# JamesKane/DecodingUsTools

Measured on AMD Instinct MI355X. Metric: reference bases classified/sec (whole node) + BED bit-exact vs CPU ref, higher is better.
Workload: dtype u8 (quality bytes thresholded to pass bits on the host, counted bit-sliced on the device); 1 GPU; coverage -L chr21 synthetic 30x 150bp paired, device-resident, one contig per GPU; contig_len=46709983, reads_per_contig=9076994, aligned_bases_per_contig=1361549100, parallelism=contig-per-gpu x1, options=cli defaults (4,500,10,20,10,1,0.1)

## Files before the change

### decodingustools_amd/csrc/pileup_rows.hip.h

```cpp
#pragma once
#include "kernels.hip.h"

namespace clk {

template <bool HEAD4> struct HeadOf { typedef uint2 type; };
template <> struct HeadOf<true> { typedef uint32_t type; };
template <bool HEAD4> __device__ __forceinline__ typename HeadOf<HEAD4>::type head_at(const void *heads, uint32_t r)
{
    return reinterpret_cast<const typename HeadOf<HEAD4>::type *>(heads)[r];
}
struct HeadCand { uint32_t cb, ce, low; bool hit; };
template <int T> __device__ __forceinline__ HeadCand head_cand(const uint2 h, uint32_t W)
{
    const uint32_t x = h.x, span = h.y & kHeadSpanMax, e = x + span;
    return HeadCand{x > W ? x - W : 0u, e - W, h.y >> 31, span && e > W && x < W + (uint32_t)T};
}
template <int T> __device__ __forceinline__ HeadCand head_cand(const uint32_t h, uint32_t W)
{
    const int32_t span = (int32_t)((h >> 16) & 0x7FFFu), dx = (int32_t)(int16_t)(uint16_t)(h - W), e = dx + span;
    return HeadCand{(uint32_t)(dx > 0 ? dx : 0), (uint32_t)e, h >> 31, span && e > 0 && dx < T};
}

typedef unsigned int RowWords __attribute__((ext_vector_type(4)));
constexpr uint32_t kRowNoUnit = 0x80000000u;
struct RowLane { __amdgpu_buffer_rsrc_t rs; uint32_t off; int32_t n; };
__device__ __forceinline__ RowLane row_lane(const uint4 *rows, const WinMeta &wm, uint32_t lane, uint32_t g0)
{
    const uint32_t s = lane >> 3;
    uint32_t n = wm.rn, first = s * wm.rn, units = 8u * wm.rn;
    if (wm.q0) {
        n = (uint32_t)(wm.q0 >> (8u * s)) & 0xFFu;
        const unsigned long long below = wm.q0 & ((1ull << (8u * s)) - 1ull);
        first = __builtin_amdgcn_sad_u8((uint32_t)below, 0u, __builtin_amdgcn_sad_u8((uint32_t)(below >> 32), 0u, 0u));
        const uint32_t lo = (uint32_t)wm.q0, hi = (uint32_t)(wm.q0 >> 32);
        const uint32_t f = (lo & 0x00FF00FFu) + ((lo >> 8) & 0x00FF00FFu) + (hi & 0x00FF00FFu) + ((hi >> 8) & 0x00FF00FFu);
        units = (f + (f >> 16)) & 0xFFFFu;
    }
    return RowLane{__builtin_amdgcn_make_buffer_rsrc(const_cast<uint4 *>(rows + (size_t)wm.rlo * 8u), 0, (int)(units * 128u), 0x00020000),
                   (first + g0) * 128u + (lane & 7u) * 16u, (int32_t)(n - g0)};
}
__device__ __forceinline__ uint4 row_unit(const RowLane &rl, int k)
{
    const RowWords v = __builtin_amdgcn_raw_buffer_load_b128(rl.rs, (k < rl.n ? rl.off : kRowNoUnit) + (uint32_t)k * 128u, 0, 0);
    return make_uint4(v.x, v.y, v.z, v.w);
}
__device__ __forceinline__ void row_advance(RowLane &rl, int by) { rl.off += (uint32_t)by * 128u; rl.n -= by; }
typedef unsigned int HeadWords __attribute__((ext_vector_type(2)));
template <bool HEAD4> __device__ __forceinline__ typename HeadOf<HEAD4>::type head_fetch(__amdgpu_buffer_rsrc_t rs, uint32_t off);
template <> __device__ __forceinline__ uint32_t head_fetch<true>(__amdgpu_buffer_rsrc_t rs, uint32_t off)
{
    return __builtin_amdgcn_raw_buffer_load_b32(rs, off, 0, 0);
}
template <> __device__ __forceinline__ uint2 head_fetch<false>(__amdgpu_buffer_rsrc_t rs, uint32_t off)
{
    const HeadWords v = __builtin_amdgcn_raw_buffer_load_b64(rs, off, 0, 0);
    return make_uint2(v.x, v.y);
}

__device__ __forceinline__ uint32_t bs_maj(uint32_t a, uint32_t b, uint32_t c) { return (a & b) | (c & (a | b)); }

template <int NP>
__device__ __forceinline__ void bs_add4(uint32_t (&c)[NP], const uint4 x)
{
    const uint32_t t0 = c[0] ^ x.x ^ x.y, k0 = bs_maj(c[0], x.x, x.y);
    c[0] = t0 ^ x.z ^ x.w;
    const uint32_t k1 = bs_maj(t0, x.z, x.w);
    uint32_t k = bs_maj(c[1], k0, k1);
    c[1] = c[1] ^ k0 ^ k1;
#pragma unroll
    for (int p = 2; p < NP; ++p) { const uint32_t t = c[p] & k; c[p] ^= k; k = t; }
}

template <int NP>
__device__ __forceinline__ uint32_t bs_less_than(const uint32_t (&c)[NP], unsigned long long K)
{
    if (NP < 64 && (K >> NP) != 0ull) return 0xFFFFFFFFu;
    uint32_t lt = 0u, eq = 0xFFFFFFFFu;
#pragma unroll
    for (int p = NP - 1; p >= 0; --p) {
        if ((K >> p) & 1ull) { lt |= eq & ~c[p]; eq &= c[p]; }
        else eq &= ~c[p];
    }
    return lt;
}

struct RowsArgs {
    const uint4    *rows;
    const void     *heads;
    const uint32_t *wide_idx;
    const WinMeta  *win;
    const uint32_t *refn;
    const uint32_t *lut8;
    uint16_t       *runs;
    uint8_t        *first_state, *last_state;
    WinPartial     *winpart;
    uint32_t        extent, n_win, n_win8;
    uint32_t        min_depth, max_depth;
    uint32_t        min_depth_for_low_mapq;
    const uint32_t *lut;
    double          max_low_mapq_fraction;
    uint8_t        *state;
    uint32_t       *dbg_raw, *dbg_qc, *dbg_low;
};

constexpr int kRowsBlock = 64;
constexpr int rows_min_waves(bool DEBUG, bool DEEP, int NP)
{
    return ((DEEP || NP > 16) ? 3 : (NP > 8 ? 4 : 5)) - (DEBUG ? 1 : 0);
}
template <int T, bool DEBUG, bool DEEP, int NP, bool HEAD4>
__global__ __launch_bounds__(kRowsBlock, rows_min_waves(DEBUG, DEEP, NP)) void k_pileup_rows(RowsArgs a)
{
    constexpr int kBlock = kRowsBlock;
    constexpr int PER = T / kBlock;
    static_assert(PER == 32 && T == 2048 && kBlock == 64, "a lane owns a block of 32 positions: T = 64 x 32, one wave");
    constexpr int kDiffWords = DEEP ? T : T / 2;
    constexpr int G = 12;
    __shared__ __attribute__((aligned(16))) uint32_t s_raw[kDiffWords];
    __shared__ __attribute__((aligned(16))) uint32_t s_low[kDiffWords];
#ifdef CL_ROWS_LDS_PAD
    __shared__ uint32_t s_pad[CL_ROWS_LDS_PAD / 4];
    s_pad[threadIdx.x] = threadIdx.x;
#endif

    const uint32_t w = (blockIdx.x & 7u) * a.n_win8 + (blockIdx.x >> 3);
    if (w >= a.n_win) return;
    const uint32_t lane = threadIdx.x;
    const uint32_t W = w * (uint32_t)T;
    const uint32_t p0 = W + lane * PER;

    const WinMeta wm = a.win[w];
    const uint32_t lo = wm.lo, hi = wm.hi, wlo = wm.wlo, wn = wm.wn;
    const uint32_t n_cand = wn + (hi - lo);
    const uint32_t ng = wm.rn;
    RowLane rl = row_lane(a.rows, wm, lane, 0u);

    uint4 rv[G];
#pragma unroll
    for (int j = 0; j < G; ++j) rv[j] = row_unit(rl, j);
    constexpr int U = 8;
    typedef typename HeadOf<HEAD4>::type Head;
    const __amdgpu_buffer_rsrc_t hrs = __builtin_amdgcn_make_buffer_rsrc(
        const_cast<char *>(static_cast<const char *>(a.heads) + (size_t)lo * sizeof(Head)), 0, (int)((hi - lo) * (uint32_t)sizeof(Head)), 0x00020000);
    auto load_heads = [&](uint32_t base, Head (&hh)[U]) {
#pragma unroll
        for (int u = 0; u < U; ++u) {
            const uint32_t o = base + (uint32_t)u * kBlock + lane - wn;
            hh[u] = head_fetch<HEAD4>(hrs, o < hi - lo ? o * (uint32_t)sizeof(Head) : 0xFFFFFFF0u);
        }
        if (wn > base) {
#pragma unroll
            for (int u = 0; u < U; ++u) {
                const uint32_t v = base + (uint32_t)u * kBlock + lane;
                if (v < wn) {
                    const uint32_t r = a.wide_idx[wlo + v];
                    __builtin_assume(r < (1u << 29));
                    hh[u] = head_at<HEAD4>(a.heads, r);
                }
            }
        }
    };
    Head hh[U];
    load_heads(0u, hh);
    const uint32_t wlut = a.lut8[lane];
    const uint32_t refn = a.refn[(size_t)w * (T / 32) + lane];

    {
        const uint4 z = make_uint4(0, 0, 0, 0);
        uint4 *r4 = reinterpret_cast<uint4 *>(s_raw), *l4 = reinterpret_cast<uint4 *>(s_low);
        const uint4 zb = DEEP ? z : make_uint4(0x8000u, 0x8000u, 0x8000u, 0x8000u);
#pragma unroll
        for (int i = 0; i < kDiffWords / 4 / kBlock; ++i) { r4[i * kBlock + lane] = zb; l4[i * kBlock + lane] = zb; }
    }
    __syncthreads();

    uint32_t c[NP];
#pragma unroll
    for (int p = 0; p < NP; ++p) c[p] = 0u;
    if (ng) {
        for (uint32_t g0 = 0; g0 < ng; g0 += (uint32_t)G) {
#pragma unroll
            for (int j = 0; j < G; ++j) {
                if (g0 + (uint32_t)j < ng) bs_add4<NP>(c, rv[j]);
            }
            if (g0 + (uint32_t)G < ng) {
                row_advance(rl, G);
#pragma unroll
                for (int j = 0; j < G; ++j) rv[j] = row_unit(rl, j);
            }
        }
    }
    for (uint32_t base = 0;;) {
#pragma unroll
        for (int u = 0; u < U; ++u) {
            const HeadCand hc = head_cand<T>(hh[u], W);
            if (hc.hit) {
                const uint32_t cb = hc.cb, ce = hc.ce;
                uint32_t ib, vb, ie, ve2;
                if (DEEP) { ib = cb; vb = 1u; ie = ce; ve2 = 0xFFFFFFFFu; }
                else {
                    ib = cb >> 1; vb = (cb & 1u) ? 0x10000u : 1u;
                    ie = ce >> 1; ve2 = (ce & 1u) ? 0xFFFF0000u : 0xFFFFFFFFu;
                }
                atomicAdd(&s_raw[ib], vb);
                if (ce < (uint32_t)T) atomicAdd(&s_raw[ie], ve2);
                if (hc.low) {
                    atomicAdd(&s_low[ib], vb);
                    if (ce < (uint32_t)T) atomicAdd(&s_low[ie], ve2);
                }
            }
        }
        base += (uint32_t)U * kBlock;
        if (base >= n_cand) break;
        load_heads(base, hh);
    }
    __syncthreads();

    const uint32_t ltb = bs_less_than<NP>(c, (unsigned long long)a.min_depth);
    const uint32_t gtb = a.max_depth > 0u ? ~bs_less_than<NP>(c, (unsigned long long)a.max_depth + 1ull) : 0u;
    unsigned long long nbits = 0;
#pragma unroll
    for (int p = 0; p < NP; ++p) nbits += (unsigned long long)__popc(c[p]) << p;

    constexpr int NH = DEEP ? 1 : PER / 2;
    uint32_t xr[NH], xl[NH];
    uint32_t tr = 0, tl = 0;
    if constexpr (DEEP) {
        xr[0] = xl[0] = 0u;
#pragma unroll
        for (int q = 0; q < PER / 4; ++q) {
            const uint4 x = reinterpret_cast<const uint4 *>(s_raw)[lane * (PER / 4) + q];
            const uint4 y = reinterpret_cast<const uint4 *>(s_low)[lane * (PER / 4) + q];
            tr += x.x + x.y + x.z + x.w; tl += y.x + y.y + y.z + y.w;
        }
    } else {
#pragma unroll
        for (int q = 0; q < NH / 4; ++q) {
            const uint4 x = reinterpret_cast<const uint4 *>(s_raw)[lane * (NH / 4) + q];
            const uint4 y = reinterpret_cast<const uint4 *>(s_low)[lane * (NH / 4) + q];
            xr[4 * q] = x.x; xr[4 * q + 1] = x.y; xr[4 * q + 2] = x.z; xr[4 * q + 3] = x.w;
            xl[4 * q] = y.x; xl[4 * q + 1] = y.y; xl[4 * q + 2] = y.z; xl[4 * q + 3] = y.w;
        }
#pragma unroll
        for (int h = 0; h < NH; ++h) {
            tr = __builtin_amdgcn_sad_u16(xr[h], 0u, tr);
            tl = __builtin_amdgcn_sad_u16(xl[h], 0u, tl);
        }
        tr = (uint32_t)(int32_t)(int16_t)(uint16_t)tr; tl = (uint32_t)(int32_t)(int16_t)(uint16_t)tl;
    }
    const uint32_t offr = dpp_incl_scan_u32(tr) - tr, offl = dpp_incl_scan_u32(tl) - tl;

    uint32_t covb = 0, lowb = 0, mx = 0;
    if constexpr (!DEEP) {
        uint32_t sr = offr, sl = offl, ncov = 0, nlow = 0;
        constexpr int B = 8;
#pragma unroll
        for (int g = 0; g < PER; g += B) {
            uint32_t r8[B], l8[B], t8[B];
#pragma unroll
            for (int k = 0; k < B; ++k) {
                const int i = g + k;
                sr += (i & 1) ? (uint32_t)((int32_t)xr[i / 2] >> 16) : (xr[i / 2] & 0xFFFFu) - 0x8000u;
                sl += (i & 1) ? (uint32_t)((int32_t)xl[i / 2] >> 16) : (xl[i / 2] & 0xFFFFu) - 0x8000u;
                r8[k] = sr; l8[k] = sl;
                t8[k] = (uint32_t)__builtin_amdgcn_ds_bpermute((int)(sr & ~3u), (int)wlut);
            }
#pragma unroll
            for (int k = 0; k < B; ++k) {
                mx = r8[k] > mx ? r8[k] : mx;
                const uint32_t thr = __builtin_amdgcn_ubfe(t8[k], r8[k] << 3, 8u);
                ncov = __builtin_amdgcn_alignbit(ncov, r8[k] - 1u, 31);
                nlow = __builtin_amdgcn_alignbit(nlow, l8[k] - thr, 31);
                if (DEBUG) {
                    if (a.dbg_raw) a.dbg_raw[p0 + g + k] = r8[k];
                    if (a.dbg_low) a.dbg_low[p0 + g + k] = l8[k];
                }
            }
        }
        covb = ~__builtin_bitreverse32(ncov); lowb = ~__builtin_bitreverse32(nlow);
    }
    if (DEEP || mx >= 255u) {
        const uint32_t mdl = a.min_depth_for_low_mapq < 0x7FFFFFFFu ? a.min_depth_for_low_mapq : 0x7FFFFFFFu;
        uint32_t sr = offr, sl = offl, ncov = 0, nlow = 0;
        mx = 0;
#pragma unroll 1
        for (int h = 0; h < PER / 2; ++h) {
            uint32_t dr[2], dl[2];
            if (DEEP) {
                dr[0] = s_raw[lane * PER + 2 * h]; dr[1] = s_raw[lane * PER + 2 * h + 1];
                dl[0] = s_low[lane * PER + 2 * h]; dl[1] = s_low[lane * PER + 2 * h + 1];
            } else {
                const uint32_t xr = s_raw[lane * (PER / 2) + h], xl = s_low[lane * (PER / 2) + h];
                dr[0] = (xr & 0xFFFFu) - 0x8000u; dr[1] = (uint32_t)((int32_t)xr >> 16);
                dl[0] = (xl & 0xFFFFu) - 0x8000u; dl[1] = (uint32_t)((int32_t)xl >> 16);
            }
#pragma unroll
            for (int k = 0; k < 2; ++k) {
                sr += dr[k]; sl += dl[k];
                const uint32_t raw = sr, low = sl;
                mx = raw > mx ? raw : mx;
                uint32_t thr = a.lut[raw < kLutSize ? raw : kLutSize - 1u];
                thr = thr < 0x7FFFFFFFu ? thr : 0x7FFFFFFFu;
                thr |= (uint32_t)((int32_t)(raw - mdl) >> 31) >> 1;
                uint32_t d = low - thr;
                if (raw >= kLutSize) {
                    const bool is_low = raw >= a.min_depth_for_low_mapq && ((double)low / (double)raw) > a.max_low_mapq_fraction;
                    d = is_low ? 0u : 0x80000000u;
                }
                ncov = __builtin_amdgcn_alignbit(ncov, raw - 1u, 31);
                nlow = __builtin_amdgcn_alignbit(nlow, d, 31);
                if (DEBUG) {
                    if (a.dbg_raw) a.dbg_raw[p0 + 2 * h + k] = raw;
                    if (a.dbg_low) a.dbg_low[p0 + 2 * h + k] = low;
                }
            }
        }
        covb = ~__builtin_bitreverse32(ncov); lowb = ~__builtin_bitreverse32(nlow);
    }
    const uint32_t n_ok = p0 >= a.extent ? 0u : (a.extent - p0 < (uint32_t)PER ? a.extent - p0 : (uint32_t)PER);
    const uint32_t okb = n_ok >= (uint32_t)PER ? 0xFFFFFFFFu : ((1u << n_ok) - 1u);
    const uint32_t Nk = refn & okb, notN = ~refn & okb, covk = covb & okb;
    const uint32_t t0 = notN & covk;
    const uint32_t rLow = t0 & lowb, t1 = t0 & ~lowb;
    const uint32_t rLT = t1 & ltb, t2 = t1 & ~ltb;
    const uint32_t rGT = t2 & gtb, rC = t2 & ~gtb;
    const uint32_t rNC = notN & ~covk;
    const uint32_t s0 = rC | rLT | rLow, s1 = rNC | rLT, s2 = rGT | rLow;
    auto state_at = [&](uint32_t j) -> uint32_t { return ((s0 >> j) & 1u) | (((s1 >> j) & 1u) << 1) | (((s2 >> j) & 1u) << 2); };
    if (DEBUG) {
#pragma unroll 1
        for (uint32_t i = 0; i < (uint32_t)PER; ++i) {
            uint32_t qc = 0;
#pragma unroll
            for (int p = 0; p < NP; ++p) qc |= ((c[p] >> i) & 1u) << p;
            if (a.dbg_qc) a.dbg_qc[p0 + i] = qc;
            a.state[p0 + i] = (uint8_t)(((okb >> i) & 1u) ? state_at(i) : 0xFFu);
        }
    }
    const uint32_t last_st = state_at((uint32_t)PER - 1u);
    const uint32_t below = (uint32_t)__shfl_up((int)last_st, 1);
    const uint32_t pv = lane > 0 ? below : state_at(0u);
    const uint32_t bnd = ((s0 ^ ((s0 << 1) | (pv & 1u))) | (s1 ^ ((s1 << 1) | ((pv >> 1) & 1u))) | (s2 ^ ((s2 << 1) | (pv >> 2)))) & okb;
    const uint32_t nb = __popc(bnd);
    {
        const uint32_t inc = dpp_incl_scan_u32(nb);
        if (nb) {
            uint16_t *dst = a.runs + (size_t)w * T + (inc - nb);
            for (uint32_t m = bnd; m; m &= m - 1u) {
                const uint32_t j = (uint32_t)__ffs((int)m) - 1u;
                *dst++ = (uint16_t)((lane * PER + j) | (state_at(j) << 12));
            }
        }
        if (lane == 0) a.first_state[w] = (uint8_t)state_at(0u);
        if (lane == kBlock - 1) a.last_state[w] = (uint8_t)last_st;
    }
    static_assert(sizeof(WinPartial) == 96 && offsetof(WinPartial, sum_reflen) == 72 && offsetof(WinPartial, n_inner) == 88 &&
                  offsetof(WinPartial, max_raw) == 92, "WinPartial as twelve 8-byte words");
    {
        const uint32_t pk0 = dpp_wave_sum_u32(__popc(Nk) | (__popc(rC) << 16));
        const uint32_t pk1 = dpp_wave_sum_u32(__popc(rNC) | (__popc(rLT) << 16));
        const uint32_t pk2 = dpp_wave_sum_u32(__popc(rGT) | (__popc(rLow) << 16));
        const uint32_t pk3 = dpp_wave_sum_u32(__popc(covk) | (nb << 16));
        const unsigned long long qc = NP <= 16 ? (unsigned long long)dpp_wave_sum_u32((uint32_t)nbits) : wave_sum_u64(nbits);
        mx = dpp_wave_max_u32(mx);
        const uint32_t f[12] = {pk0 & 0xFFFFu, pk0 >> 16, pk1 & 0xFFFFu, pk1 >> 16, pk2 & 0xFFFFu, pk2 >> 16,
                                pk3 & 0xFFFFu, (uint32_t)qc, 0u, 0u, 0u, pk3 >> 16};
        if (lane < 12u) {
            uint32_t vlo = 0u;
#pragma unroll
            for (uint32_t k = 0; k < 12u; ++k) vlo = lane == k ? f[k] : vlo;
            const uint32_t vhi = lane == 7u ? (uint32_t)(qc >> 32) : (lane == 11u ? mx : 0u);
            reinterpret_cast<unsigned long long *>(a.winpart + w)[lane] = (unsigned long long)vlo | ((unsigned long long)vhi << 32);
        }
    }
}

}
```

Before: 758.8 billion bases/s.

## Pack raw and low-MAPQ diffs into one word and use CSA tree counters

```diff
diff --git a/decodingustools_amd/csrc/pileup_rows.hip.h b/decodingustools_amd/csrc/pileup_rows.hip.h
--- a/decodingustools_amd/csrc/pileup_rows.hip.h
+++ b/decodingustools_amd/csrc/pileup_rows.hip.h
@@ -69,6 +69,37 @@
     c[1] = c[1] ^ k0 ^ k1;
 #pragma unroll
     for (int p = 2; p < NP; ++p) { const uint32_t t = c[p] & k; c[p] ^= k; k = t; }
+}
+
+__device__ __forceinline__ uint32_t bs_csa(uint32_t &s, uint32_t a, uint32_t b)
+{
+    const uint32_t k = bs_maj(s, a, b);
+    s ^= a ^ b;
+    return k;
+}
+template <int NP>
+__device__ __forceinline__ void bs_ripple(uint32_t (&c)[NP], int from, uint32_t k)
+{
+#pragma unroll
+    for (int p = from; p < NP; ++p) { const uint32_t t = c[p] & k; c[p] ^= k; k = t; }
+}
+template <int NP>
+__device__ __forceinline__ void bs_add8(uint32_t (&c)[NP], const uint4 x, const uint4 y)
+{
+    static_assert(NP >= 4, "the tree of 8 rows ends in plane 2");
+    const uint32_t a0 = bs_csa(c[0], x.x, x.y), a1 = bs_csa(c[0], x.z, x.w), a2 = bs_csa(c[0], y.x, y.y), a3 = bs_csa(c[0], y.z, y.w);
+    const uint32_t b0 = bs_csa(c[1], a0, a1), b1 = bs_csa(c[1], a2, a3);
+    bs_ripple<NP>(c, 3, bs_csa(c[2], b0, b1));
+}
+template <int NP>
+__device__ __forceinline__ void bs_add16(uint32_t (&c)[NP], const uint4 x, const uint4 y, const uint4 z, const uint4 v)
+{
+    static_assert(NP >= 5, "the tree of 16 rows ends in plane 3");
+    const uint32_t a0 = bs_csa(c[0], x.x, x.y), a1 = bs_csa(c[0], x.z, x.w), a2 = bs_csa(c[0], y.x, y.y), a3 = bs_csa(c[0], y.z, y.w);
+    const uint32_t a4 = bs_csa(c[0], z.x, z.y), a5 = bs_csa(c[0], z.z, z.w), a6 = bs_csa(c[0], v.x, v.y), a7 = bs_csa(c[0], v.z, v.w);
+    const uint32_t b0 = bs_csa(c[1], a0, a1), b1 = bs_csa(c[1], a2, a3), b2 = bs_csa(c[1], a4, a5), b3 = bs_csa(c[1], a6, a7);
+    const uint32_t d0 = bs_csa(c[2], b0, b1), d1 = bs_csa(c[2], b2, b3);
+    bs_ripple<NP>(c, 4, bs_csa(c[3], d0, d1));
 }
 
 template <int NP>
@@ -106,7 +137,7 @@
 constexpr int kRowsBlock = 64;
 constexpr int rows_min_waves(bool DEBUG, bool DEEP, int NP)
 {
-    return ((DEEP || NP > 16) ? 3 : (NP > 8 ? 4 : 5)) - (DEBUG ? 1 : 0);
+    return ((DEEP || NP > 16) ? 3 : (NP > 8 ? 4 : 5)) - (DEBUG ? (!DEEP && NP <= 8 ? 2 : 1) : 0);
 }
 template <int T, bool DEBUG, bool DEEP, int NP, bool HEAD4>
 __global__ __launch_bounds__(kRowsBlock, rows_min_waves(DEBUG, DEEP, NP)) void k_pileup_rows(RowsArgs a)
@@ -114,10 +145,9 @@
     constexpr int kBlock = kRowsBlock;
     constexpr int PER = T / kBlock;
     static_assert(PER == 32 && T == 2048 && kBlock == 64, "a lane owns a block of 32 positions: T = 64 x 32, one wave");
-    constexpr int kDiffWords = DEEP ? T : T / 2;
     constexpr int G = 12;
-    __shared__ __attribute__((aligned(16))) uint32_t s_raw[kDiffWords];
-    __shared__ __attribute__((aligned(16))) uint32_t s_low[kDiffWords];
+    __shared__ __attribute__((aligned(16))) uint32_t s_diff[DEEP ? 2 * T : T];
+    uint32_t *const s_raw = s_diff, *const s_low = s_diff + T;
 #ifdef CL_ROWS_LDS_PAD
     __shared__ uint32_t s_pad[CL_ROWS_LDS_PAD / 4];
     s_pad[threadIdx.x] = threadIdx.x;
@@ -166,11 +196,9 @@
     const uint32_t refn = a.refn[(size_t)w * (T / 32) + lane];
 
     {
-        const uint4 z = make_uint4(0, 0, 0, 0);
-        uint4 *r4 = reinterpret_cast<uint4 *>(s_raw), *l4 = reinterpret_cast<uint4 *>(s_low);
-        const uint4 zb = DEEP ? z : make_uint4(0x8000u, 0x8000u, 0x8000u, 0x8000u);
-#pragma unroll
-        for (int i = 0; i < kDiffWords / 4 / kBlock; ++i) { r4[i * kBlock + lane] = zb; l4[i * kBlock + lane] = zb; }
+        uint4 *d4 = reinterpret_cast<uint4 *>(s_diff);
+#pragma unroll
+        for (int i = 0; i < (DEEP ? 2 * T : T) / 4 / kBlock; ++i) d4[i * kBlock + lane] = make_uint4(0, 0, 0, 0);
     }
     __syncthreads();
 
@@ -180,8 +208,9 @@
     if (ng) {
         for (uint32_t g0 = 0; g0 < ng; g0 += (uint32_t)G) {
 #pragma unroll
-            for (int j = 0; j < G; ++j) {
-                if (g0 + (uint32_t)j < ng) bs_add4<NP>(c, rv[j]);
+            for (int j = 0; j < G; j += 4) {
+                if (g0 + (uint32_t)j + 2u < ng) bs_add16<NP>(c, rv[j], rv[j + 1], rv[j + 2], rv[j + 3]);
+                else if (g0 + (uint32_t)j < ng) bs_add8<NP>(c, rv[j], rv[j + 1]);
             }
             if (g0 + (uint32_t)G < ng) {
                 row_advance(rl, G);
@@ -196,17 +225,17 @@
             const HeadCand hc = head_cand<T>(hh[u], W);
             if (hc.hit) {
                 const uint32_t cb = hc.cb, ce = hc.ce;
-                uint32_t ib, vb, ie, ve2;
-                if (DEEP) { ib = cb; vb = 1u; ie = ce; ve2 = 0xFFFFFFFFu; }
-                else {
-                    ib = cb >> 1; vb = (cb & 1u) ? 0x10000u : 1u;
-                    ie = ce >> 1; ve2 = (ce & 1u) ? 0xFFFF0000u : 0xFFFFFFFFu;
-                }
-                atomicAdd(&s_raw[ib], vb);
-                if (ce < (uint32_t)T) atomicAdd(&s_raw[ie], ve2);
-                if (hc.low) {
-                    atomicAdd(&s_low[ib], vb);
-                    if (ce < (uint32_t)T) atomicAdd(&s_low[ie], ve2);
+                if (DEEP) {
+                    atomicAdd(&s_raw[cb], 1u);
+                    if (ce < (uint32_t)T) atomicAdd(&s_raw[ce], 0xFFFFFFFFu);
+                    if (hc.low) {
+                        atomicAdd(&s_low[cb], 1u);
+                        if (ce < (uint32_t)T) atomicAdd(&s_low[ce], 0xFFFFFFFFu);
+                    }
+                } else {
+                    const uint32_t v = 1u + (hc.low << 16);
+                    atomicAdd(&s_diff[cb], v);
+                    if (ce < (uint32_t)T) atomicAdd(&s_diff[ce], 0u - v);
                 }
             }
         }
@@ -222,61 +251,58 @@
 #pragma unroll
     for (int p = 0; p < NP; ++p) nbits += (unsigned long long)__popc(c[p]) << p;
 
-    constexpr int NH = DEEP ? 1 : PER / 2;
-    uint32_t xr[NH], xl[NH];
+    constexpr int NX = DEEP ? 1 : PER;
+    uint32_t x[NX];
     uint32_t tr = 0, tl = 0;
     if constexpr (DEEP) {
-        xr[0] = xl[0] = 0u;
+        x[0] = 0u;
 #pragma unroll
         for (int q = 0; q < PER / 4; ++q) {
-            const uint4 x = reinterpret_cast<const uint4 *>(s_raw)[lane * (PER / 4) + q];
-            const uint4 y = reinterpret_cast<const uint4 *>(s_low)[lane * (PER / 4) + q];
-            tr += x.x + x.y + x.z + x.w; tl += y.x + y.y + y.z + y.w;
+            const uint4 xq = reinterpret_cast<const uint4 *>(s_raw)[lane * (PER / 4) + q];
+            const uint4 yq = reinterpret_cast<const uint4 *>(s_low)[lane * (PER / 4) + q];
+            tr += xq.x + xq.y + xq.z + xq.w; tl += yq.x + yq.y + yq.z + yq.w;
         }
     } else {
 #pragma unroll
-        for (int q = 0; q < NH / 4; ++q) {
-            const uint4 x = reinterpret_cast<const uint4 *>(s_raw)[lane * (NH / 4) + q];
-            const uint4 y = reinterpret_cast<const uint4 *>(s_low)[lane * (NH / 4) + q];
-            xr[4 * q] = x.x; xr[4 * q + 1] = x.y; xr[4 * q + 2] = x.z; xr[4 * q + 3] = x.w;
-            xl[4 * q] = y.x; xl[4 * q + 1] = y.y; xl[4 * q + 2] = y.z; xl[4 * q + 3] = y.w;
-        }
-#pragma unroll
-        for (int h = 0; h < NH; ++h) {
-            tr = __builtin_amdgcn_sad_u16(xr[h], 0u, tr);
-            tl = __builtin_amdgcn_sad_u16(xl[h], 0u, tl);
-        }
-        tr = (uint32_t)(int32_t)(int16_t)(uint16_t)tr; tl = (uint32_t)(int32_t)(int16_t)(uint16_t)tl;
-    }
-    const uint32_t offr = dpp_incl_scan_u32(tr) - tr, offl = dpp_incl_scan_u32(tl) - tl;
+        for (int q = 0; q < NX / 4; ++q) {
+            const uint4 xq = reinterpret_cast<const uint4 *>(s_diff)[lane * (NX / 4) + q];
+            x[4 * q] = xq.x; x[4 * q + 1] = xq.y; x[4 * q + 2] = xq.z; x[4 * q + 3] = xq.w;
+        }
+#pragma unroll
+        for (int i = 0; i < NX; ++i) tr += x[i];
+    }
+    const uint32_t offr = dpp_incl_scan_u32(tr) - tr;
+    uint32_t offl = 0u;
+    if constexpr (DEEP) offl = dpp_incl_scan_u32(tl) - tl;
 
     uint32_t covb = 0, lowb = 0, mx = 0;
     if constexpr (!DEEP) {
-        uint32_t sr = offr, sl = offl, ncov = 0, nlow = 0;
+        uint32_t s = offr, ncov = 0, nlow = 0;
+        int32_t mc = -0x10000;
         constexpr int B = 8;
 #pragma unroll
         for (int g = 0; g < PER; g += B) {
-            uint32_t r8[B], l8[B], t8[B];
+            uint32_t s8[B], t8[B];
 #pragma unroll
             for (int k = 0; k < B; ++k) {
-                const int i = g + k;
-                sr += (i & 1) ? (uint32_t)((int32_t)xr[i / 2] >> 16) : (xr[i / 2] & 0xFFFFu) - 0x8000u;
-                sl += (i & 1) ? (uint32_t)((int32_t)xl[i / 2] >> 16) : (xl[i / 2] & 0xFFFFu) - 0x8000u;
-                r8[k] = sr; l8[k] = sl;
-                t8[k] = (uint32_t)__builtin_amdgcn_ds_bpermute((int)(sr & ~3u), (int)wlut);
+                s += x[g + k];
+                s8[k] = s;
+                t8[k] = (uint32_t)__builtin_amdgcn_ds_bpermute((int)s, (int)wlut);
             }
 #pragma unroll
             for (int k = 0; k < B; ++k) {
-                mx = r8[k] > mx ? r8[k] : mx;
-                const uint32_t thr = __builtin_amdgcn_ubfe(t8[k], r8[k] << 3, 8u);
-                ncov = __builtin_amdgcn_alignbit(ncov, r8[k] - 1u, 31);
-                nlow = __builtin_amdgcn_alignbit(nlow, l8[k] - thr, 31);
+                const uint32_t thr = __builtin_amdgcn_alignbyte(t8[k], t8[k], s8[k]) & 0xFFu;
+                const uint32_t dc = (s8[k] << 16) - 0x10000u;
+                mc = (int32_t)dc > mc ? (int32_t)dc : mc;
+                ncov = __builtin_amdgcn_alignbit(ncov, dc, 31);
+                nlow = __builtin_amdgcn_alignbit(nlow, (s8[k] >> 16) - thr, 31);
                 if (DEBUG) {
-                    if (a.dbg_raw) a.dbg_raw[p0 + g + k] = r8[k];
-                    if (a.dbg_low) a.dbg_low[p0 + g + k] = l8[k];
+                    if (a.dbg_raw) a.dbg_raw[p0 + g + k] = s8[k] & 0xFFFFu;
+                    if (a.dbg_low) a.dbg_low[p0 + g + k] = s8[k] >> 16;
                 }
             }
         }
+        mx = ((uint32_t)mc + 0x10000u) >> 16;
         covb = ~__builtin_bitreverse32(ncov); lowb = ~__builtin_bitreverse32(nlow);
     }
     if (DEEP || mx >= 255u) {
@@ -290,14 +316,13 @@
                 dr[0] = s_raw[lane * PER + 2 * h]; dr[1] = s_raw[lane * PER + 2 * h + 1];
                 dl[0] = s_low[lane * PER + 2 * h]; dl[1] = s_low[lane * PER + 2 * h + 1];
             } else {
-                const uint32_t xr = s_raw[lane * (PER / 2) + h], xl = s_low[lane * (PER / 2) + h];
-                dr[0] = (xr & 0xFFFFu) - 0x8000u; dr[1] = (uint32_t)((int32_t)xr >> 16);
-                dl[0] = (xl & 0xFFFFu) - 0x8000u; dl[1] = (uint32_t)((int32_t)xl >> 16);
+                dr[0] = s_diff[lane * PER + 2 * h]; dr[1] = s_diff[lane * PER + 2 * h + 1];
+                dl[0] = dl[1] = 0u;
             }
 #pragma unroll
             for (int k = 0; k < 2; ++k) {
                 sr += dr[k]; sl += dl[k];
-                const uint32_t raw = sr, low = sl;
+                const uint32_t raw = DEEP ? sr : sr & 0xFFFFu, low = DEEP ? sl : sr >> 16;
                 mx = raw > mx ? raw : mx;
                 uint32_t thr = a.lut[raw < kLutSize ? raw : kLutSize - 1u];
                 thr = thr < 0x7FFFFFFFu ? thr : 0x7FFFFFFFu;
```

Result: faster. 836.1 billion bases/s, median of 6 (+10.2%).
